# sashakolpakov/graphem-rapids

Measured on AMD Instinct MI355X. Metric: layout iterations/s, higher is better.
Workload: dtype f32

## Files before the change

graphem-rapids_amd/_native.py:

```python
import ctypes
import os

import numpy as np

_HERE = os.path.dirname(os.path.abspath(__file__))
LIB_PATH = os.path.join(_HERE, "libgraphem_hip.so")

GH_OK, GH_ERR_INVALID, GH_ERR_RUNTIME, GH_ERR_K_TOO_LARGE, GH_ERR_HIP, GH_ERR_NOMEM = range(6)

SYMBOLS = [
    "gh_create", "gh_destroy", "gh_last_error", "gh_set_positions", "gh_get_positions", "gh_positions_device",
    "gh_row_stride", "gh_step", "gh_run", "gh_sync", "gh_spring_forces", "gh_knn_midpoints",
    "gh_intersection_forces", "gh_integrate_normalise", "gh_step_begin", "gh_knn_partial_device", "gh_knn_partial_cols", "gh_knn_merged_device", "gh_rows_packed_device", "gh_step_unpack_rows", "gh_set_packed_rows", "gh_step_merge",
    "gh_stats_partial_device", "gh_step_finish", "gh_timing_enable", "gh_timing_reset", "gh_timing_count",
    "gh_timing_get", "gh_device_count", "gh_version", "gh_knn_last_counts", "gh_set_stream",
    "gh_positions_rows_allocated", "gh_knn_points", "gh_stats_rows", "gh_spmv_symnorm",
    "gh_spectral_last_error", "gh_gather_layout", "gh_gather_buffer_device", "gh_gather_slot_bytes",
    "gh_step_finish_gathered", "gh_vertex_order", "gh_positions_unpadded_device", "gh_radial_topk",
    "gh_comm_unique_id", "gh_comm_init_rccl", "gh_loopback_group_create", "gh_loopback_group_destroy",
    "gh_comm_init_loopback", "gh_comm_destroy", "gh_run_partitioned", "gh_comm_last_error", "gh_debug_stamps",
    "gh_knn_cdist_stats", "gh_rank_layout", "gh_step_finish_own", "gh_comm_available", "gh_selftest_arith",
    "gh_create_f64", "gh_set_positions_f64", "gh_get_positions_f64", "gh_positions_device_f64", "gh_spring_forces_f64",
    "gh_intersection_forces_f64", "gh_trlan_sweep", "gh_knn_ivf_config", "gh_knn_ivf_list_sizes",
    "gh_torch_randperm_prefix", "gh_torch_randperm_isa", "gh_run_torch_sampled", "gh_set_cdist_replay", "gh_sampler_stats",
    "gh_overlap_layout", "gh_rows_all_device", "gh_rows_all_row_floats", "gh_stats_all_device", "gh_stats_all_block_doubles", "gh_step_rows_early",
    "gh_step_pack_rows", "gh_step_finish_overlap",
    "gh_ic_create", "gh_ic_destroy", "gh_ic_last_error", "gh_ic_arc_count", "gh_ic_set_memory_budget", "gh_ic_spread",
]


class GhParams(ctypes.Structure):
    _fields_ = [("L_min", ctypes.c_float), ("k_attr", ctypes.c_float), ("k_inter", ctypes.c_float),
                ("n_neighbors", ctypes.c_int32), ("sample_size", ctypes.c_int32), ("seed", ctypes.c_uint64),
                ("reorder", ctypes.c_int32), ("knn_method", ctypes.c_int32), ("knn_distance", ctypes.c_int32),
                ("ivf_lists", ctypes.c_int32), ("ivf_probes", ctypes.c_int32)]


REORDER = {"auto": 0, "off": 1, "bfs": 2}
KNN_METHOD = {"auto": 0, "scan": 1, "grid": 2, "ivf": 3}
KNN_DISTANCE = {"exact": 0, "cdist": 1}


class GhPartition(ctypes.Structure):
    _fields_ = [("row_lo", ctypes.c_int64), ("row_hi", ctypes.c_int64),
                ("edge_lo", ctypes.c_int64), ("edge_hi", ctypes.c_int64), ("edge_rule", ctypes.c_int32)]


EDGES_RANGE, EDGES_HASHED = 0, 1


_lib = None


def load():
    global _lib
    if _lib is not None:
        return _lib
    global LIB_PATH
    if os.environ.get("GRAPHEM_HIP_LIB"):
        LIB_PATH = os.environ["GRAPHEM_HIP_LIB"]
    if not os.path.exists(LIB_PATH):
        raise RuntimeError(
            f"{LIB_PATH} is missing: build it with `python graphem-rapids_amd/build.py` "
            "(hipcc --offload-arch=gfx950). The HIP backend has no CPU fallback.")
# ... 109 lines not shown
    L.gh_trlan_sweep.restype = ctypes.c_int
    L.gh_spectral_last_error.argtypes = []
    L.gh_spectral_last_error.restype = ctypes.c_char_p
    L.gh_stats_rows.argtypes = [vp]
    L.gh_stats_rows.restype = i32
    L.gh_knn_points.argtypes = [ctypes.c_int, vp, i64, vp, i64, i32, i32, vp]
    L.gh_knn_points.restype = ctypes.c_int
    L.gh_knn_last_counts.argtypes = [vp, vp, vp, vp]
    L.gh_knn_last_counts.restype = ctypes.c_int
    L.gh_knn_cdist_stats.argtypes = [vp, vp, vp]
    L.gh_knn_cdist_stats.restype = ctypes.c_int
    L.gh_sampler_stats.argtypes = [vp, vp]
    L.gh_sampler_stats.restype = ctypes.c_int
    L.gh_set_cdist_replay.argtypes = [vp, i32]
    L.gh_set_cdist_replay.restype = ctypes.c_int
    L.gh_knn_ivf_config.argtypes = [vp, vp, vp]
    L.gh_knn_ivf_config.restype = ctypes.c_int
    L.gh_knn_ivf_list_sizes.argtypes = [vp, vp, ctypes.c_int32]
    L.gh_knn_ivf_list_sizes.restype = ctypes.c_int
    L.gh_comm_unique_id.argtypes = [vp]
    L.gh_comm_unique_id.restype = ctypes.c_int
    L.gh_comm_init_rccl.argtypes = [vp, i32, i32, vp]
    L.gh_comm_init_rccl.restype = ctypes.c_int
    L.gh_loopback_group_create.argtypes = [i32]
    L.gh_loopback_group_create.restype = vp
    L.gh_loopback_group_destroy.argtypes = [vp]
    L.gh_loopback_group_destroy.restype = None
    L.gh_comm_init_loopback.argtypes = [vp, vp, i32]
    L.gh_comm_init_loopback.restype = ctypes.c_int
    L.gh_comm_destroy.argtypes = [vp]
# ... 283 lines not shown
        return self.lib.gh_stats_partial_device(self.handle)

    def knn_last_counts(self):
        a, b, c = (np.zeros(self.S, dtype=np.int32) for _ in range(3))
        self._chk(self.lib.gh_knn_last_counts(self.handle, ptr(a), ptr(b), ptr(c)))
        return a, b, c

    def knn_cdist_stats(self):
        a, b = ctypes.c_int32(0), ctypes.c_int32(0)
        self._chk(self.lib.gh_knn_cdist_stats(self.handle, ctypes.byref(a), ctypes.byref(b)))
        return a.value, b.value

    def set_cdist_replay(self, all_ties):
        self._chk(self.lib.gh_set_cdist_replay(self.handle, 1 if all_ties else 0))

    def knn_ivf_config(self):
        a, b = ctypes.c_int32(0), ctypes.c_int32(0)
        self._chk(self.lib.gh_knn_ivf_config(self.handle, ctypes.byref(a), ctypes.byref(b)))
        return a.value, b.value

    def knn_ivf_list_sizes(self):
        out = np.zeros(self.knn_ivf_config()[0], dtype=np.int32)
        self._chk(self.lib.gh_knn_ivf_list_sizes(self.handle, ptr(out), len(out)))
        return out

    def timing_enable(self, on=True):
        self._chk(self.lib.gh_timing_enable(self.handle, 1 if on else 0))

    def timing_reset(self):
        self._chk(self.lib.gh_timing_reset(self.handle))
# ... 105 lines not shown
```

graphem-rapids_amd/csrc/api.hip:

```cpp
#include "common.h"
#include "engine.h"

#include "torch_randperm.h"

#include <algorithm>
#include <chrono>
#include <condition_variable>
#include <mutex>
#include <new>
#include <thread>
#include <stdlib.h>
#include <string.h>

static thread_local std::string g_create_error;
void gh_set_create_error(const std::string &msg) { g_create_error = msg; }

gh_scope::gh_scope(gh_engine *h_, const char *name, hipStream_t on) : h(h_), stream(on ? on : h_->stream) {
    if (!h->timing) return;
    for (size_t i = 0; i < h->timers.size(); ++i)
        if (h->timers[i].name == name) slot = (int)i;
    if (slot < 0) {
        h->timers.emplace_back();
        h->timers.back().name = name;
        slot = (int)h->timers.size() - 1;
// ... 49 lines not shown
    }
    return GH_OK;
}

static gh_status reject_f64(gh_engine *h, const char *what) {
    if (!h->f64) return GH_OK;
    h->err = std::string(what) + " is not available on a float64 engine";
    return GH_ERR_INVALID;
}

static void free_all(gh_engine *h) {
    gh_f64_free(h);
    gh_ivf_free(h);
    void *ptrs[] = {h->d_edges, h->d_rowptr, h->d_adj, h->d_pos, (h->d_gbuf || h->d_rows_all) ? (void *)h->d_new_own : (void *)h->d_new, h->d_gbuf, h->d_rows_all, h->d_rows_pk, h->d_stats_all, h->d_tmpF, h->d_tmpF2, h->d_io, h->d_acc,
                    h->d_tflag, h->d_touched, h->d_tcount, h->d_sampled, h->d_q, h->d_qscan, h->d_qA, h->d_qexact, h->d_order, h->d_long_rows, h->d_long_ownptr, h->d_long_ownadj, h->d_long_eptr, h->d_long_erow, h->d_long_terms, h->d_own_long, h->d_cand, h->d_cnt,
                    h->d_ovf, h->d_sel_redo, h->d_tq_count, h->d_tq_base, h->d_tq_touched, h->d_dbg_cnt, h->d_partial, h->d_merged, h->d_first_edge, h->d_own_eids, h->d_mid, h->d_Fs, h->d_gmin, h->d_sub_uv, h->d_stamps, h->d_tau_flag, h->d_wait_failed, h->d_grid_u32, h->d_grid_smid, h->d_grid_temp, h->d_stats_comb, h->d_rows_packed, h->d_rare, h->d_cd_rows, h->d_cd_vbuf, h->d_cd_cmin, h->d_cd_stat, h->d_vblock, h->d_blockstats, (h->d_gbuf || h->d_rows_all) ? (void *)h->d_stats_own : (void *)h->d_stats, h->d_iscratch, h->d_stream_ids};
    for (void *p : ptrs)
        if (p) (void)hipFree(p);
    if (h->h_ring) (void)hipHostFree(h->h_ring);
    for (hipEvent_t e : h->ring_ev)
        if (e) (void)hipEventDestroy(e);
    if (h->own_stream) (void)hipStreamDestroy(h->own_stream);
}

gh_status gh_check_create_args(int device_id, int64_t n, int32_t D, int64_t E, const int32_t *edges, const gh_params *params,
                               int f64_max_D, double f64_k_attr) {
    auto fail = [&](gh_status st, const std::string &msg) { g_create_error = msg; return st; };
    const bool f64 = f64_max_D > 0;
    if (n <= 0) return fail(GH_ERR_INVALID, "Adjacency matrix cannot be empty");
    if (D <= 0) return fail(GH_ERR_INVALID, "Number of components must be positive, got " + std::to_string(D));
    if (f64 && D > f64_max_D) return fail(GH_ERR_INVALID, "the float64 engine takes up to " + std::to_string(f64_max_D) + " components");
// ... 97 lines not shown
    if (!up(h->d_edges, g.edges, sizeof(int32_t) * 2 * (size_t)E) || !up32(h->d_rowptr, g.rowptr) ||
        !up(h->d_adj, g.adj.data(), sizeof(int32_t) * (size_t)h->adj_len) || !up32(h->d_first_edge, g.first_edge) ||
        !up32(h->d_vblock, g.vblock) || (hashed && !up32(h->d_own_eids, g.own_eids)) ||
        (h->nlong && (!up32(h->d_long_rows, g.long_rows) || !up32(h->d_long_ownptr, g.long_ownptr) ||
                      !up32(h->d_long_eptr, g.long_eptr) || !up32(h->d_long_erow, g.long_erow) ||
                      !up32(h->d_long_ownadj, g.long_ownadj) || !up(h->d_own_long, g.own_long.data(), g.own_long.size()))) ||
        hipStreamSynchronize(h->stream) != hipSuccess) {
        h->err = "upload of the graph failed";
        return GH_ERR_HIP;
    }
    GH_TRY(gh_grid_alloc(h));
    GH_TRY(gh_ivf_alloc(h));
    GH_TRY(gh_cdist_alloc(h));
    GH_A(d_tau_flag, 1, true);
    GH_A(d_wait_failed, 1, true);
    if (sw.stamps) GH_A(d_stamps, ((size_t)std::max(h->n_vblocks, 1) + GH_STAMP_EXTRA) * 8, true);
#undef GH_A
    if (h->thr_M1 > 0 && hipMemcpy(h->d_sub_uv, g.sub_uv.data(), sizeof(int32_t) * g.sub_uv.size(), hipMemcpyHostToDevice) != hipSuccess) {
        h->err = "upload of the threshold subset failed";
        return GH_ERR_HIP;
    }
    if (!h->order_host.empty()) {
        GH_TRY(dev_alloc(h, &h->d_order, (size_t)n, false));
        if (hipMemcpy(h->d_order, h->order_host.data(), sizeof(int32_t) * (size_t)n, hipMemcpyHostToDevice) != hipSuccess) {
            h->err = "upload of the vertex order failed";
            return GH_ERR_HIP;
        }
    }
    return GH_OK;
}
// ... 29 lines not shown
    h->rows = h->part.row_hi - h->part.row_lo;

    auto bail = [&](gh_status st) { g_create_error = h->err; free_all(h); delete h; return st; };
    if (hipSetDevice(device_id) != hipSuccess) return bail(GH_ERR_HIP);
    if (hipStreamCreateWithFlags(&h->own_stream, hipStreamNonBlocking) != hipSuccess) { h->err = "hipStreamCreate failed"; return bail(GH_ERR_HIP); }
    h->stream = h->own_stream;
    h->pos_rows = n + GH_POS_PAD_ROWS;
    const create_switches sw = read_switches();
    h->opt_no_presetup = sw.no_presetup;

    gh_graph_plan g;
    gh_plan_graph(h, edges, part != nullptr, sw.reorder ? atoi(sw.reorder) : params->reorder, &g);
    if (auto_method) gh_auto_knn_method(h);
    gh_choose_threshold_subset(h);
    gh_plan_threshold_subset(h, &g);
    h->tau_embedded = sw.tau_separate >= 0 ? sw.tau_separate == 0 : h->n_vblocks <= 2048;

    const gh_status st = allocate_and_upload(h, g, sw);
    if (st != GH_OK) return bail(st);
    *out = h;
    return GH_OK;
}

extern "C" void gh_destroy(gh_handle h) {
    if (!h) return;
    (void)hipSetDevice(h->device);
    (void)hipStreamSynchronize(h->stream);
    resolve_timers(h);
    gh_comm_free(h);
    free_all(h);
    delete h;
// ... 8 lines not shown
    gh_set_lookahead(h, nullptr);
    GH_HIP(hipMemcpyAsync(h->d_io, pos, sizeof(float) * (size_t)h->n * h->D, hipMemcpyHostToDevice, h->stream));
    GH_TRY(gh_launch_pad(h, h->d_io, h->d_pos));
    GH_HIP(hipStreamSynchronize(h->stream));
    return GH_OK;
}

static gh_status download_padded(gh_engine *h, const float *d_src, float *host) {
    GH_TRY(gh_launch_unpad(h, d_src, h->d_io));
    GH_HIP(hipMemcpyAsync(host, h->d_io, sizeof(float) * (size_t)h->n * h->D, hipMemcpyDeviceToHost, h->stream));
    GH_HIP(hipStreamSynchronize(h->stream));
    return GH_OK;
}

static gh_status check_device_waits(gh_engine *h) {
    if (!h->tau_embedded || !h->d_wait_failed) return GH_OK;
    int32_t failed = 0;
    GH_HIP(hipMemcpyAsync(&failed, h->d_wait_failed, sizeof(failed), hipMemcpyDeviceToHost, h->stream));
    GH_HIP(hipStreamSynchronize(h->stream));
    if (failed) {
        GH_HIP(hipMemsetAsync(h->d_wait_failed, 0, sizeof(int32_t), h->stream));
        GH_HIP(hipStreamSynchronize(h->stream));
        h->tau_embedded = false;
        h->err = "a workgroup of the fused spring+scan launch timed out waiting for the thresholds of its own launch; "
                 "results since the last successful gh_sync / gh_get_positions are invalid -- set the positions again. "
                 "The engine now computes the thresholds in a launch of their own (as GRAPHEM_HIP_TAU_SEPARATE=1 does); "
                 "please report this";
        return GH_ERR_RUNTIME;
    }
    return GH_OK;
}

extern "C" gh_status gh_get_positions(gh_handle h, float *pos) {
    GH_TRY(check_handle(h));
    if (h->f64) return pos ? gh_f64_get_positions_f32(h, pos) : GH_ERR_INVALID;
    if (!pos) { h->err = "positions is NULL"; return GH_ERR_INVALID; }
    GH_TRY(check_device_waits(h));
    return download_padded(h, h->d_pos, pos);
// ... 159 lines not shown
    if (iters == 0) return GH_OK;
    GH_TRY(check_whole(h, "gh_run"));
    GH_TRY(check_k(h));
    int32_t *d_ids = nullptr;
    GH_TRY(gh_upload_sample_stream(h, iters, sample_stream, &d_ids));
    const gh_ids own = gh_own_ids(h);
    auto src = [&](int32_t t) { return d_ids ? gh_ids{GH_IDS_GIVEN, d_ids + (size_t)t * h->S} : own; };
    return run_iterations(h, iters, d_ids == nullptr, src, nothing_before);
}

extern "C" gh_status gh_set_cdist_replay(gh_handle h, int32_t all_ties) {
    GH_TRY(check_handle(h));
    GH_TRY(reject_f64(h, "gh_set_cdist_replay"));
    if (!h->cdist) { h->err = "gh_set_cdist_replay: not a GH_DIST_CDIST engine"; return GH_ERR_INVALID; }
    h->cd_all_ties = all_ties != 0;
    return GH_OK;
}

extern "C" gh_status gh_torch_randperm_prefix(uint8_t *rng_state, int64_t state_bytes, int64_t n, int64_t S, int32_t iters,
                                              int32_t *ids) {
    if (!rng_state || state_bytes != GH_TORCH_RNG_STATE_BYTES || n < 0 || n >= ((int64_t)1 << 31) || S < 0 || S > n || iters < 0 ||
        (!ids && iters > 0 && S > 0))
        return GH_ERR_INVALID;
    gh_mt19937 mt;
    if (!gh_mt_load(&mt, rng_state)) return GH_ERR_INVALID;
    std::vector<int64_t> scratch((size_t)gh_rp_scratch_words(S));
    for (int32_t t = 0; t < iters; ++t) gh_torch_randperm_prefix_one(&mt, n, S, ids + (size_t)t * (size_t)S, scratch.data());
    gh_mt_store(&mt, rng_state);
    return GH_OK;
}
// ... 481 lines not shown
```

graphem-rapids_amd/csrc/engine.h:

```cpp
#pragma once
#include <hip/hip_runtime.h>
#include <stdint.h>
#include <string>
#include <vector>

#include "../../include/graphem_hip.h"

#define GH_CAND_CAP 16384
#define GH_SEL_BUF 4096
#define GH_SEL_CHUNK 2048
#define GH_CNT_STRIDE 32
#define GH_POS_PAD_ROWS 1024
inline int gh_fix_blocks(int LD) { return LD <= 16 ? 2 * LD : 0; }
#define GH_SCAN_MIN_EDGES 16384

struct gh_timer_slot {
    std::string name;
    double total_ms = 0.0;
    int64_t launches = 0;
    std::vector<std::pair<hipEvent_t, hipEvent_t>> pending;
};

enum { GH_IDS_GIVEN = 0, GH_IDS_SAMPLER = 1, GH_IDS_ARANGE = 2 };
struct gh_ids {
// ... 129 lines not shown

    int grid_G = 0, grid_bits = 0;
    int64_t grid_cells = 0;
    size_t grid_temp_bytes = 0;
    uint32_t *d_grid_u32 = nullptr;
    void *d_grid_smid = nullptr;
    void *d_grid_temp = nullptr;

    gh_ivf *ivf = nullptr;

    double *d_blockstats = nullptr;
    int nblocks_update = 0;
    double *d_stats = nullptr;

    bool tau_embedded = false;
    unsigned *d_tau_flag = nullptr;
    int32_t *d_wait_failed = nullptr;

#define GH_STAMP_EXTRA 8192
    unsigned long long *d_stamps = nullptr;
    bool timing = false;
    std::vector<gh_timer_slot> timers;
};

inline gh_ids gh_own_ids(const gh_engine *h) { return gh_ids{h->S >= h->E ? GH_IDS_ARANGE : GH_IDS_SAMPLER, h->d_sampled}; }
inline void gh_set_lookahead(gh_engine *h, const gh_ids *next) {
    h->lookahead.valid = next != nullptr;
    if (next) { h->lookahead.src = *next; h->lookahead.iter = h->iter + 1; }
}

struct gh_scope {
// ... 50 lines not shown
                               int D, int K, uint64_t *d_keys, std::string *err);
gh_status gh_cdist_alloc(gh_engine *h);
gh_status gh_knn_merge_cdist(gh_engine *h, const uint64_t *gathered, int world);
gh_status gh_knn_finish_cdist(gh_engine *h, bool all_rows, bool fuse_intersect);
bool gh_grid_path(const gh_engine *h);
gh_status gh_grid_alloc(gh_engine *h);
gh_status gh_grid_search(gh_engine *h);
bool gh_ivf_path(const gh_engine *h);
gh_status gh_ivf_alloc(gh_engine *h);
void gh_ivf_free(gh_engine *h);
gh_status gh_ivf_search(gh_engine *h);
gh_status gh_radial_topk_device(gh_engine *h, int K, uint64_t *d_part, int nparts, int32_t *d_ids);
int gh_fused_mfma_kb(const gh_engine *h);
bool gh_fused_uses_mfma(const gh_engine *h);
int gh_fused_tile(const gh_engine *h);
gh_status gh_launch_spring_scan(gh_engine *h);
gh_status gh_knn_merge(gh_engine *h, const uint64_t *gathered, int world);
gh_status gh_launch_intersect(gh_engine *h);
gh_status gh_launch_inter_cleanup(gh_engine *h);
gh_status gh_launch_spring_mid(gh_engine *h);
gh_status gh_launch_mid_only(gh_engine *h);
gh_status gh_launch_integrate(gh_engine *h);
gh_status gh_launch_spring_only(gh_engine *h, float *d_F);
gh_status gh_launch_inter_to_dense(gh_engine *h, float *d_F);
gh_status gh_launch_integrate_given(gh_engine *h, const float *d_Fs, const float *d_Fi);
gh_status gh_launch_normalise(gh_engine *h, bool with_cleanup, const gh_ids *next = nullptr);
gh_status gh_launch_normalise_gathered(gh_engine *h, const gh_ids *next);
gh_status gh_launch_normalise_own(gh_engine *h, const double *stats_all, int world);
gh_status gh_launch_unpack_rows(gh_engine *h);
struct gh_long_args;
// ... 37 lines not shown
```

graphem-rapids_amd/csrc/fused.hip:

```cpp
#include "common.h"
#include "engine.h"
#include "scan_core.h"
#include "tau_core.h"

#include <stdio.h>
#include <stdlib.h>

static bool fused_mfma(int LD, int D, int64_t S) {
    (void)S;
    return D <= 16 && (LD == 4 || LD == 8 || LD == 16);
}
static int fused_mfma_kb(int LD, int D, int64_t S) { return fused_mfma(LD, D, S) && D <= 3 ? 0 : -1; }
static void fused_cfg(int LD, int D, int64_t S, int64_t own_edges, int *nt, int *r) {
    (void)LD; (void)D; (void)S; (void)own_edges;
    *nt = 256;
    *r = 2;
}
bool gh_fused_uses_mfma(const gh_engine *h) { return h->fused_scan && fused_mfma(h->LD, h->D, h->S); }
int gh_fused_mfma_kb(const gh_engine *h) { return h->fused_scan ? fused_mfma_kb(h->LD, h->D, h->S) : -1; }
int gh_fused_tile(const gh_engine *h) {
    int nt, r;
    fused_cfg(h->LD, h->D, h->S, h->own_count, &nt, &r);
    return nt * r;
}

namespace {

template <int D, int LD, int NT, bool LONG>
__device__ __forceinline__ void gh_phase_a(const float *__restrict__ pos, const int32_t *__restrict__ rowptr,
                                           const int32_t *__restrict__ adj, const int32_t *__restrict__ first_edge,
                                           int v0, int v1, int fe0, int nedges, int64_t row_lo, float L_min, float neg_k,
                                           float *__restrict__ Fs, float *__restrict__ out_new, float *mids,
                                           double (&sx)[LD], double (&sxx)[LD], const gh_long_args &la,
                                           const float *__restrict__ Fpre = nullptr ) {
// ... 210 lines not shown
        const int nb_ = nbad;
        for (int p = threadIdx.x; p < nb_ * nq; p += NT) {
            const int s = p % nq;
            const gh_h8 hi = qa[2 * s + 1];
            if ((float)hi[4] == GH_MF_NEVER) continue;
            park(s_lo, s, badlist[p / nq]);
        }
    }
    __syncthreads();
    GH_STAMP(4);
    gh_flush_hits<HITBUF, NT>(hkey, hq, &hcount, cand, cnt);
    GH_STAMP(5);
#undef GH_STAMP
}

template <int D, int LD, bool LONG>
__global__ __launch_bounds__(256) void spring_scan_mfmaw_kernel(
    const float *__restrict__ pos, const int32_t *__restrict__ rowptr, const int32_t *__restrict__ adj,
    const int32_t *__restrict__ first_edge, const int32_t *__restrict__ own_eids,
    const int32_t *__restrict__ vblock, int64_t row_lo, float L_min, float neg_k, float *__restrict__ Fs,
    float *__restrict__ out_new, double *__restrict__ blockstats, const float *__restrict__ qt,
    const float *__restrict__ qscan, int S,
    uint64_t *__restrict__ cand, int32_t *__restrict__ cnt, gh_long_args la, gh_tau_args ta,
    unsigned long long *__restrict__ stamps) {
    constexpr int NT = 256, R = 2, TILE = NT * R, NB = 2 * R;
    constexpr int HITBUF = LD == 16 ? 256 : 512;
    constexpr int KB = D <= 10 ? 1 : 2;
    constexpr int QS = LD + 4, QT = LD;
    if ((int)blockIdx.x < ta.nblocks) {
        if (blockIdx.y == 0) gh_tau_produce<NT, -1>(ta, stamps ? stamps + ((int64_t)gridDim.x - 2 * ta.nblocks + GH_STAMP_EXTRA + blockIdx.x) * 8 : nullptr);
// ... 195 lines not shown
    ta.cdist = h->cdist ? 1 : 0;
    ta.flag = h->d_tau_flag;
    ta.target = (unsigned)h->S;
    ta.nblocks = gh_tau_blocks((int)h->S, nt);
    ta.wait_failed = h->d_wait_failed;
    return ta;
}

template <int D, int R, bool DEFER>
void launch_mfma_d(gh_engine *h) {
    const gh_tau_args ta = fused_tau_args(h, 256);
    spring_scan_mfma_kernel<D, R, DEFER><<<dim3(fused_grid(h, ta)), dim3(256), 0, h->stream>>>(
        h->d_pos, h->d_rowptr, h->d_adj, h->d_first_edge, h->d_own_eids, h->d_vblock, h->part.row_lo, h->prm.L_min,
        -h->prm.k_attr, h->d_Fs, h->d_new, h->d_blockstats, h->d_q, reinterpret_cast<const gh_h8 *>(h->d_qA),
        h->d_qexact, (int)h->S, h->d_cand, h->d_cnt, gh_make_long_args(h, true), ta, h->d_stamps);
}
template <int D, int R>
void launch_mfma(gh_engine *h) {
    if (R == 2 && h->n_vblocks <= 2048) launch_mfma_d<D, R, (R == 2)>(h);
    else launch_mfma_d<D, R, false>(h);
}

template <int D, int LD, bool LONG>
void launch_mfmaw_l(gh_engine *h) {
    unsigned ny = 1;
    if (h->n_vblocks < 384) {
        static int resident = 0;
        if (resident == 0) {
            int occ = 0, cus = 0;
            if (hipOccupancyMaxActiveBlocksPerMultiprocessor(&occ, spring_scan_mfmaw_kernel<D, LD, LONG>, 256, 0) != hipSuccess) occ = 1;
// ... 27 lines not shown
        switch (h->D) {
            case 4: launch_mfmaw<4, 4>(h); break;
            case 5: launch_mfmaw<5, 8>(h); break;
            case 6: launch_mfmaw<6, 8>(h); break;
            case 7: launch_mfmaw<7, 8>(h); break;
            case 8: launch_mfmaw<8, 8>(h); break;
            case 9: launch_mfmaw<9, 16>(h); break;
            case 10: launch_mfmaw<10, 16>(h); break;
            case 11: launch_mfmaw<11, 16>(h); break;
            case 12: launch_mfmaw<12, 16>(h); break;
            case 13: launch_mfmaw<13, 16>(h); break;
            case 14: launch_mfmaw<14, 16>(h); break;
            case 15: launch_mfmaw<15, 16>(h); break;
            default: launch_mfmaw<16, 16>(h); break;
        }
    } else if (fused_mfma(h->LD, h->D, h->S)) {
        if (h->D == 2) launch_mfma<2, 2>(h); else launch_mfma<3, 2>(h);
    } else {
        h->err = "fused spring+scan launched for an unsupported dimension";
        return GH_ERR_RUNTIME;
    }
    GH_LAUNCH_CHECK();
    h->new0_ready = true;
    return GH_OK;
}
```

include/graphem_hip.h:

```cpp
#ifndef GRAPHEM_HIP_H
#define GRAPHEM_HIP_H

#include <stdint.h>

#ifdef __cplusplus
extern "C" {
#endif

typedef struct gh_engine *gh_handle;

typedef enum {
    GH_OK = 0,
    GH_ERR_INVALID = 1,
    GH_ERR_RUNTIME = 2,
    GH_ERR_K_TOO_LARGE = 3,
    GH_ERR_HIP = 4,
    GH_ERR_NOMEM = 5
} gh_status;

typedef struct {
    float L_min;
    float k_attr;
    float k_inter;
    int32_t n_neighbors;
// ... 107 lines not shown
gh_status gh_run_partitioned(gh_handle h, int32_t iters, const int32_t *sample_stream);
const char *gh_comm_last_error(void);


gh_status gh_timing_enable(gh_handle h, int32_t on);
gh_status gh_timing_reset(gh_handle h);
int32_t gh_timing_count(gh_handle h);
gh_status gh_timing_get(gh_handle h, int32_t i, const char **name, double *total_ms, int64_t *launches);


gh_status gh_debug_stamps(gh_handle h, unsigned long long *out, int64_t count);

gh_status gh_knn_last_counts(gh_handle h, int32_t *subset_counts, int32_t *final_counts, int32_t *overflow);
gh_status gh_knn_cdist_stats(gh_handle h, int32_t *full_pass_rows, int32_t *unresolved_tie_rows);
gh_status gh_set_cdist_replay(gh_handle h, int32_t all_ties);
gh_status gh_knn_ivf_config(gh_handle h, int32_t *lists, int32_t *probes);
gh_status gh_knn_ivf_list_sizes(gh_handle h, int32_t *sizes, int32_t count);

gh_status gh_knn_points(int device_id, const float *q, int64_t nq, const float *ref, int64_t nref,
                        int32_t n_components, int32_t k, int64_t *out);

gh_status gh_radial_topk(gh_handle h, int32_t k, int32_t *ids);

gh_status gh_spmv_symnorm(void *hip_stream, int64_t n, const int64_t *indptr, const int32_t *indices,
                          const double *inv_sqrt_deg, const double *x, double *y);
gh_status gh_trlan_sweep(void *hip_stream, int64_t n, const int64_t *indptr, const int32_t *indices,
                         const double *inv_sqrt_deg, double *V, int32_t nl, int32_t m, int32_t k, double *Td,
                         double *work, double *beta, double *hmax);
const char *gh_spectral_last_error(void);

// ... 21 lines not shown
```

Baseline: 6062.

## Add query-cell spatial filter to fused spring+scan kernel

Adds a fused spring+scan kernel variant. Block 0 builds a small 8-per-axis grid of quantile-bounded cells over the sampled queries and publishes it to global memory. Every other workgroup waits on an epoch flag, loads the table into shared memory, and tests each midpoint only against the queries listed in its cell plus a 'wide' list, instead of running the split-f16 MFMA pre-filter against all queries. It is picked automatically when tau is not embedded and D<=3, S<=256. It adds a cross-workgroup spin-wait with a timeout fallback, and it risks imbalance when many queries land in the wide list.

```diff
diff --git a/graphem-rapids_amd/_native.py b/graphem-rapids_amd/_native.py
--- a/graphem-rapids_amd/_native.py
+++ b/graphem-rapids_amd/_native.py
@@ -22,7 +22,7 @@
     "gh_knn_cdist_stats", "gh_rank_layout", "gh_step_finish_own", "gh_comm_available", "gh_selftest_arith",
     "gh_create_f64", "gh_set_positions_f64", "gh_get_positions_f64", "gh_positions_device_f64", "gh_spring_forces_f64",
     "gh_intersection_forces_f64", "gh_trlan_sweep", "gh_knn_ivf_config", "gh_knn_ivf_list_sizes",
-    "gh_torch_randperm_prefix", "gh_torch_randperm_isa", "gh_run_torch_sampled", "gh_set_cdist_replay", "gh_sampler_stats",
+    "gh_torch_randperm_prefix", "gh_torch_randperm_isa", "gh_run_torch_sampled", "gh_set_cdist_replay", "gh_set_scan_filter", "gh_get_scan_filter", "gh_qcell_probe", "gh_sampler_stats",
     "gh_overlap_layout", "gh_rows_all_device", "gh_rows_all_row_floats", "gh_stats_all_device", "gh_stats_all_block_doubles", "gh_step_rows_early",
     "gh_step_pack_rows", "gh_step_finish_overlap",
     "gh_ic_create", "gh_ic_destroy", "gh_ic_last_error", "gh_ic_arc_count", "gh_ic_set_memory_budget", "gh_ic_spread",
@@ -48,6 +48,8 @@
 
 EDGES_RANGE, EDGES_HASHED = 0, 1
 
+
+SCAN_FILTERS = {"auto": 0, "mfma": 1, "cells": 2}
 
 _lib = None
 
@@ -187,6 +189,12 @@
     L.gh_sampler_stats.restype = ctypes.c_int
     L.gh_set_cdist_replay.argtypes = [vp, i32]
     L.gh_set_cdist_replay.restype = ctypes.c_int
+    L.gh_set_scan_filter.argtypes = [vp, i32]
+    L.gh_set_scan_filter.restype = ctypes.c_int
+    L.gh_get_scan_filter.argtypes = [vp, ctypes.POINTER(i32)]
+    L.gh_get_scan_filter.restype = ctypes.c_int
+    L.gh_qcell_probe.argtypes = [vp, i32, vp, vp, vp, i64, vp, vp]
+    L.gh_qcell_probe.restype = ctypes.c_int
     L.gh_knn_ivf_config.argtypes = [vp, vp, vp]
     L.gh_knn_ivf_config.restype = ctypes.c_int
     L.gh_knn_ivf_list_sizes.argtypes = [vp, vp, ctypes.c_int32]
@@ -500,6 +508,14 @@
     def set_cdist_replay(self, all_ties):
         self._chk(self.lib.gh_set_cdist_replay(self.handle, 1 if all_ties else 0))
 
+    def set_scan_filter(self, mode):
+        self._chk(self.lib.gh_set_scan_filter(self.handle, SCAN_FILTERS[mode]))
+
+    def scan_filter(self):
+        v = ctypes.c_int32(0)
+        self._chk(self.lib.gh_get_scan_filter(self.handle, ctypes.byref(v)))
+        return {b: a for a, b in SCAN_FILTERS.items()}[v.value]
+
     def knn_ivf_config(self):
         a, b = ctypes.c_int32(0), ctypes.c_int32(0)
         self._chk(self.lib.gh_knn_ivf_config(self.handle, ctypes.byref(a), ctypes.byref(b)))
diff --git a/graphem-rapids_amd/csrc/api.hip b/graphem-rapids_amd/csrc/api.hip
--- a/graphem-rapids_amd/csrc/api.hip
+++ b/graphem-rapids_amd/csrc/api.hip
@@ -1,5 +1,6 @@
 #include "common.h"
 #include "engine.h"
+#include "qcell_core.h"
 
 #include "torch_randperm.h"
 
@@ -87,7 +88,7 @@
     gh_ivf_free(h);
     void *ptrs[] = {h->d_edges, h->d_rowptr, h->d_adj, h->d_pos, (h->d_gbuf || h->d_rows_all) ? (void *)h->d_new_own : (void *)h->d_new, h->d_gbuf, h->d_rows_all, h->d_rows_pk, h->d_stats_all, h->d_tmpF, h->d_tmpF2, h->d_io, h->d_acc,
                     h->d_tflag, h->d_touched, h->d_tcount, h->d_sampled, h->d_q, h->d_qscan, h->d_qA, h->d_qexact, h->d_order, h->d_long_rows, h->d_long_ownptr, h->d_long_ownadj, h->d_long_eptr, h->d_long_erow, h->d_long_terms, h->d_own_long, h->d_cand, h->d_cnt,
-                    h->d_ovf, h->d_sel_redo, h->d_tq_count, h->d_tq_base, h->d_tq_touched, h->d_dbg_cnt, h->d_partial, h->d_merged, h->d_first_edge, h->d_own_eids, h->d_mid, h->d_Fs, h->d_gmin, h->d_sub_uv, h->d_stamps, h->d_tau_flag, h->d_wait_failed, h->d_grid_u32, h->d_grid_smid, h->d_grid_temp, h->d_stats_comb, h->d_rows_packed, h->d_rare, h->d_cd_rows, h->d_cd_vbuf, h->d_cd_cmin, h->d_cd_stat, h->d_vblock, h->d_blockstats, (h->d_gbuf || h->d_rows_all) ? (void *)h->d_stats_own : (void *)h->d_stats, h->d_iscratch, h->d_stream_ids};
+                    h->d_ovf, h->d_sel_redo, h->d_tq_count, h->d_tq_base, h->d_tq_touched, h->d_dbg_cnt, h->d_partial, h->d_merged, h->d_first_edge, h->d_own_eids, h->d_mid, h->d_Fs, h->d_gmin, h->d_sub_uv, h->d_stamps, h->d_tau_flag, h->d_wait_failed, h->d_qcell, h->d_qc_flag, h->d_grid_u32, h->d_grid_smid, h->d_grid_temp, h->d_stats_comb, h->d_rows_packed, h->d_rare, h->d_cd_rows, h->d_cd_vbuf, h->d_cd_cmin, h->d_cd_stat, h->d_vblock, h->d_blockstats, (h->d_gbuf || h->d_rows_all) ? (void *)h->d_stats_own : (void *)h->d_stats, h->d_iscratch, h->d_stream_ids};
     for (void *p : ptrs)
         if (p) (void)hipFree(p);
     if (h->h_ring) (void)hipHostFree(h->h_ring);
@@ -215,6 +216,8 @@
     GH_TRY(gh_cdist_alloc(h));
     GH_A(d_tau_flag, 1, true);
     GH_A(d_wait_failed, 1, true);
+    GH_A(d_qcell, GH_QC_WORDS, true);
+    GH_A(d_qc_flag, 1, true);
     if (sw.stamps) GH_A(d_stamps, ((size_t)std::max(h->n_vblocks, 1) + GH_STAMP_EXTRA) * 8, true);
 #undef GH_A
     if (h->thr_M1 > 0 && hipMemcpy(h->d_sub_uv, g.sub_uv.data(), sizeof(int32_t) * g.sub_uv.size(), hipMemcpyHostToDevice) != hipSuccess) {
@@ -274,7 +277,8 @@
     if (auto_method) gh_auto_knn_method(h);
     gh_choose_threshold_subset(h);
     gh_plan_threshold_subset(h, &g);
-    h->tau_embedded = sw.tau_separate >= 0 ? sw.tau_separate == 0 : h->n_vblocks <= 2048;
+    h->tau_embedded_plan = sw.tau_separate >= 0 ? sw.tau_separate == 0 : h->n_vblocks <= 2048;
+    gh_choose_scan_filter(h);
 
     const gh_status st = allocate_and_upload(h, g, sw);
     if (st != GH_OK) return bail(st);
@@ -313,14 +317,24 @@
 }
 
 static gh_status check_device_waits(gh_engine *h) {
-    if (!h->tau_embedded || !h->d_wait_failed) return GH_OK;
+    if (!(h->tau_embedded || h->qcells) || !h->d_wait_failed) return GH_OK;
     int32_t failed = 0;
     GH_HIP(hipMemcpyAsync(&failed, h->d_wait_failed, sizeof(failed), hipMemcpyDeviceToHost, h->stream));
     GH_HIP(hipStreamSynchronize(h->stream));
     if (failed) {
         GH_HIP(hipMemsetAsync(h->d_wait_failed, 0, sizeof(int32_t), h->stream));
         GH_HIP(hipStreamSynchronize(h->stream));
-        h->tau_embedded = false;
+        if (h->qcells) {
+            h->scan_filter = GH_FILTER_MFMA;
+            gh_choose_scan_filter(h);
+            h->lookahead.valid = false;
+            h->err = "a workgroup of the fused spring+scan launch timed out waiting for the query-cell table of its own "
+                     "launch; results since the last successful gh_sync / gh_get_positions are invalid -- set the positions "
+                     "again.  The engine now uses the split-f16 pre-filter (GH_FILTER_MFMA); please report this";
+            return GH_ERR_RUNTIME;
+        }
+        h->tau_embedded_plan = false;
+        gh_choose_scan_filter(h);
         h->err = "a workgroup of the fused spring+scan launch timed out waiting for the thresholds of its own launch; "
                  "results since the last successful gh_sync / gh_get_positions are invalid -- set the positions again. "
                  "The engine now computes the thresholds in a launch of their own (as GRAPHEM_HIP_TAU_SEPARATE=1 does); "
@@ -510,6 +524,52 @@
     GH_TRY(reject_f64(h, "gh_set_cdist_replay"));
     if (!h->cdist) { h->err = "gh_set_cdist_replay: not a GH_DIST_CDIST engine"; return GH_ERR_INVALID; }
     h->cd_all_ties = all_ties != 0;
+    return GH_OK;
+}
+
+extern "C" gh_status gh_set_scan_filter(gh_handle h, int32_t mode) {
+    GH_TRY(check_handle(h));
+    GH_TRY(reject_f64(h, "gh_set_scan_filter"));
+    if (mode != GH_FILTER_AUTO && mode != GH_FILTER_MFMA && mode != GH_FILTER_CELLS) {
+        h->err = "gh_set_scan_filter: mode must be GH_FILTER_AUTO, GH_FILTER_MFMA or GH_FILTER_CELLS";
+        return GH_ERR_INVALID;
+    }
+    if (mode == GH_FILTER_CELLS && !gh_fused_cells_ok(h)) {
+        h->err = "gh_set_scan_filter: the query-cell filter needs a fused engine with n_components <= 3 and 1 <= sample_size <= " +
+                 std::to_string(GH_QC_SMAX);
+        return GH_ERR_INVALID;
+    }
+    h->scan_filter = mode;
+    const bool was_embedded = h->tau_embedded;
+    gh_choose_scan_filter(h);
+    if (h->tau_embedded != was_embedded) h->lookahead.valid = false;
+    return GH_OK;
+}
+
+extern "C" gh_status gh_get_scan_filter(gh_handle h, int32_t *mode) {
+    GH_TRY(check_handle(h));
+    if (!mode) { h->err = "mode is NULL"; return GH_ERR_INVALID; }
+    *mode = h->f64 || !gh_fused_uses_mfma(h) || h->D > 3 ? GH_FILTER_AUTO : h->qcells ? GH_FILTER_CELLS : GH_FILTER_MFMA;
+    return GH_OK;
+}
+
+extern "C" gh_status gh_qcell_probe(const float *bounds, int32_t D, const float *q, const float *tau, const float *m, int64_t n,
+                                    float *d2, int32_t *cells) {
+    if (!bounds || !q || !tau || !m || !d2 || !cells || D < 1 || D > 3 || n < 0) return GH_ERR_INVALID;
+    for (int64_t i = 0; i < n; ++i) {
+        float acc = 0.0f;
+        for (int d = 0; d < D; ++d) {
+            const float df = q[i * D + d] - m[i * D + d];
+            acc = fmaf(df, df, acc);
+            const float *b = bounds + d * (GH_QC_G - 1);
+            int lo, hi;
+            gh_qc_axis_box(b, q[i * D + d], tau[i], lo, hi);
+            cells[(i * D + d) * 3] = gh_qc_axis_cell(b, m[i * D + d]);
+            cells[(i * D + d) * 3 + 1] = lo;
+            cells[(i * D + d) * 3 + 2] = hi;
+        }
+        d2[i] = acc;
+    }
     return GH_OK;
 }
 
diff --git a/graphem-rapids_amd/csrc/engine.h b/graphem-rapids_amd/csrc/engine.h
--- a/graphem-rapids_amd/csrc/engine.h
+++ b/graphem-rapids_amd/csrc/engine.h
@@ -167,7 +167,13 @@
     double *d_stats = nullptr;
 
     bool tau_embedded = false;
+    bool tau_embedded_plan = false;
     unsigned *d_tau_flag = nullptr;
+    int scan_filter = 0;
+    bool qcells = false;
+    uint32_t *d_qcell = nullptr;
+    unsigned *d_qc_flag = nullptr;
+    unsigned qc_epoch = 0;
     int32_t *d_wait_failed = nullptr;
 
 #define GH_STAMP_EXTRA 8192
@@ -248,6 +254,8 @@
 int gh_fused_mfma_kb(const gh_engine *h);
 bool gh_fused_uses_mfma(const gh_engine *h);
 int gh_fused_tile(const gh_engine *h);
+bool gh_fused_cells_ok(const gh_engine *h);
+void gh_choose_scan_filter(gh_engine *h);
 gh_status gh_launch_spring_scan(gh_engine *h);
 gh_status gh_knn_merge(gh_engine *h, const uint64_t *gathered, int world);
 gh_status gh_launch_intersect(gh_engine *h);
diff --git a/graphem-rapids_amd/csrc/fused.hip b/graphem-rapids_amd/csrc/fused.hip
--- a/graphem-rapids_amd/csrc/fused.hip
+++ b/graphem-rapids_amd/csrc/fused.hip
@@ -1,5 +1,6 @@
 #include "common.h"
 #include "engine.h"
+#include "qcell_core.h"
 #include "scan_core.h"
 #include "tau_core.h"
 
@@ -17,7 +18,15 @@
     *r = 2;
 }
 bool gh_fused_uses_mfma(const gh_engine *h) { return h->fused_scan && fused_mfma(h->LD, h->D, h->S); }
-int gh_fused_mfma_kb(const gh_engine *h) { return h->fused_scan ? fused_mfma_kb(h->LD, h->D, h->S) : -1; }
+int gh_fused_mfma_kb(const gh_engine *h) { return h->fused_scan && !h->qcells ? fused_mfma_kb(h->LD, h->D, h->S) : -1; }
+bool gh_fused_cells_ok(const gh_engine *h) {
+    return h->fused_scan && fused_mfma(h->LD, h->D, h->S) && h->D <= 3 && h->S >= 1 && h->S <= GH_QC_SMAX;
+}
+void gh_choose_scan_filter(gh_engine *h) {
+    const bool want = h->scan_filter == GH_FILTER_CELLS || (h->scan_filter == GH_FILTER_AUTO && !h->tau_embedded_plan);
+    h->qcells = want && gh_fused_cells_ok(h);
+    h->tau_embedded = h->tau_embedded_plan && !h->qcells;
+}
 int gh_fused_tile(const gh_engine *h) {
     int nt, r;
     fused_cfg(h->LD, h->D, h->S, h->own_count, &nt, &r);
@@ -258,6 +267,145 @@
 #undef GH_STAMP
 }
 
+template <int D>
+__global__ __launch_bounds__(256) void spring_scan_cells_kernel(
+    const float *__restrict__ pos, const int32_t *__restrict__ rowptr, const int32_t *__restrict__ adj,
+    const int32_t *__restrict__ first_edge, const int32_t *__restrict__ own_eids,
+    const int32_t *__restrict__ vblock, int64_t row_lo, float L_min, float neg_k, float *__restrict__ Fs,
+    float *__restrict__ out_new, double *__restrict__ blockstats, const float *__restrict__ qt, int S,
+    uint32_t *__restrict__ qcell, unsigned *__restrict__ qc_flag, unsigned epoch, int32_t *__restrict__ wait_failed,
+    uint64_t *__restrict__ cand, int32_t *__restrict__ cnt, gh_long_args la, int cdist, unsigned long long *__restrict__ stamps) {
+    constexpr int LD = 4, NT = 256, R = 2, TILE = NT * R, HITBUF = 512;
+    static_assert(D <= 3, "query records of one 16-byte load");
+    __shared__ float4 tile[TILE];
+    __shared__ float4 qrec[GH_QC_SMAX];
+    __shared__ uint32_t tab[GH_QC_WORDS];
+    __shared__ uint64_t hkey[HITBUF];
+    __shared__ int hq[HITBUF];
+    __shared__ uint32_t ids[TILE];
+    __shared__ int hcount;
+    if (blockIdx.x == 0) {
+        gh_qc_build<D, NT>(reinterpret_cast<const float4 *>(qt), S, tab, qrec, reinterpret_cast<uint32_t *>(hkey));
+        for (int i = threadIdx.x; i < GH_QC_WORDS; i += NT)
+            __hip_atomic_store(qcell + i, tab[i], __ATOMIC_RELAXED, __HIP_MEMORY_SCOPE_AGENT);
+        asm volatile("s_waitcnt vmcnt(0)" ::: "memory");
+        __syncthreads();
+        if (threadIdx.x == 0) __hip_atomic_store(qc_flag, epoch, __ATOMIC_RELAXED, __HIP_MEMORY_SCOPE_AGENT);
+        return;
+    }
+    const int nbx = (int)gridDim.x - 1;
+    const int bx = (int)blockIdx.x - 1;
+#define GH_STAMP(k) do { if (stamps && threadIdx.x == 0) stamps[(int64_t)bx * 8 + (k)] = wall_clock64(); } while (0)
+    GH_STAMP(0);
+    if (stamps && threadIdx.x == 0) { stamps[(int64_t)bx * 8 + 6] = vblock[bx + 1] - vblock[bx]; stamps[(int64_t)bx * 8 + 7] = first_edge[vblock[bx + 1]] - first_edge[vblock[bx]]; }
+    float *mids = reinterpret_cast<float *>(tile);
+    const int v0 = vblock[bx], v1 = vblock[bx + 1];
+    const int fe0 = first_edge[v0];
+    const int nedges = first_edge[v1] - fe0;
+    if (threadIdx.x == 0) hcount = 0;
+    for (int j = threadIdx.x; j < nedges; j += NT) ids[j] = own_eids ? (uint32_t)own_eids[fe0 + j] : (uint32_t)(fe0 + j);
+
+    const int t_idle = min(NT, (v1 - v0 + 63) / 64 * 64);
+    auto stage = [&](int t0) {
+        for (int i = (int)threadIdx.x - t0; i < S; i += NT - t0) qrec[i] = reinterpret_cast<const float4 *>(qt)[i];
+        unsigned spins = 0;
+        while ((int)(__hip_atomic_load(qc_flag, __ATOMIC_RELAXED, __HIP_MEMORY_SCOPE_AGENT) - epoch) < 0) {
+            __builtin_amdgcn_s_sleep(32);
+            if (++spins > (1u << 20)) { *wait_failed = 1; break; }
+        }
+        __builtin_amdgcn_fence(__ATOMIC_ACQUIRE, "wavefront");
+        for (int i = (int)threadIdx.x - t0; i < GH_QC_WORDS / 4; i += NT - t0)
+            reinterpret_cast<float4 *>(tab)[i] = gh_ld_f4(reinterpret_cast<const float4 *>(qcell) + i, true);
+    };
+    if (t_idle < NT && (int)threadIdx.x >= t_idle) stage(t_idle);
+
+    __shared__ double red[(NT / 64) * 2 * LD];
+    {
+        double sx[LD], sxx[LD];
+        gh_phase_a<D, LD, NT, true>(pos, rowptr, adj, first_edge, v0, v1, fe0, nedges, row_lo, L_min, neg_k, Fs, out_new, mids, sx, sxx, la);
+        GH_STAMP(1);
+        gh_block_stats<LD, NT>(sx, sxx, red, blockstats, bx, nbx, v1 - v0);
+    }
+    GH_STAMP(2);
+    if (t_idle == NT) {
+        stage(0);
+        __syncthreads();
+    }
+    GH_STAMP(3);
+
+    const float *bnd = reinterpret_cast<const float *>(tab + GH_QC_OFF_B);
+    const uint16_t *ptr = reinterpret_cast<const uint16_t *>(tab + GH_QC_OFF_PTR);
+    const uint8_t *ent = reinterpret_cast<const uint8_t *>(tab + GH_QC_OFF_ENT);
+    const uint8_t *wide = reinterpret_cast<const uint8_t *>(tab + GH_QC_OFF_WIDE);
+    const int nwide = (int)tab[GH_QC_OFF_NWIDE];
+    auto park = [&](int s, const float4 qr, int j, const float (&m)[3]) {
+        const float q[3] = {qr.x, qr.y, qr.z};
+        float d2 = 0.0f;
+#pragma unroll
+        for (int d = 0; d < D; ++d) {
+            const float df = q[d] - m[d];
+            d2 = fmaf(df, df, d2);
+        }
+        if (d2 <= qr.w) {
+            if (cdist) d2 = gh_aten_cdist<D>(q, m);
+            const uint32_t id = ids[j];
+            const int p = atomicAdd(&hcount, 1);
+            if (p < HITBUF) { hkey[p] = gh_key(d2, id); hq[p] = s; }
+            else gh_append_candidate(cand, cnt, s, gh_key(d2, id));
+        }
+    };
+    constexpr int U = 4;
+    float m[R][3];
+    int e[R], e1[R];
+#pragma unroll
+    for (int r = 0; r < R; ++r) {
+        const int j = (int)threadIdx.x + r * NT;
+        const float4 mv = tile[j < nedges ? j : 0];
+        m[r][0] = mv.x; m[r][1] = mv.y; m[r][2] = mv.z;
+        int c = gh_qc_axis_cell(bnd, m[r][0]) + GH_QC_G * gh_qc_axis_cell(bnd + 8, m[r][1]);
+        if constexpr (D == 3) c += GH_QC_G * GH_QC_G * gh_qc_axis_cell(bnd + 16, m[r][2]);
+        e[r] = j < nedges ? ptr[c] : 0;
+        e1[r] = j < nedges ? ptr[c + 1] : 0;
+    }
+#pragma unroll
+    for (int r = 0; r < R; ++r) {
+        const int j = (int)threadIdx.x + r * NT;
+        for (int b = e[r]; b < e1[r]; b += U) {
+            int s[U];
+            float4 qr[U];
+#pragma unroll
+            for (int u = 0; u < U; ++u) s[u] = ent[min(b + u, e1[r] - 1)];
+#pragma unroll
+            for (int u = 0; u < U; ++u) qr[u] = qrec[s[u]];
+#pragma unroll
+            for (int u = 0; u < U; ++u)
+                if (b + u < e1[r]) park(s[u], qr[u], j, m[r]);
+        }
+    }
+    for (int b = 0; b < nwide; b += U) {
+        int s[U];
+        float4 qr[U];
+#pragma unroll
+        for (int u = 0; u < U; ++u) s[u] = wide[min(b + u, nwide - 1)];
+#pragma unroll
+        for (int u = 0; u < U; ++u) qr[u] = qrec[s[u]];
+#pragma unroll
+        for (int r = 0; r < R; ++r) {
+            const int j = (int)threadIdx.x + r * NT;
+            if (j < nedges) {
+#pragma unroll
+                for (int u = 0; u < U; ++u)
+                    if (b + u < nwide) park(s[u], qr[u], j, m[r]);
+            }
+        }
+    }
+    __syncthreads();
+    GH_STAMP(4);
+    gh_flush_hits<HITBUF, NT>(hkey, hq, &hcount, cand, cnt);
+    GH_STAMP(5);
+#undef GH_STAMP
+}
+
 template <int D, int LD, bool LONG>
 __global__ __launch_bounds__(256) void spring_scan_mfmaw_kernel(
     const float *__restrict__ pos, const int32_t *__restrict__ rowptr, const int32_t *__restrict__ adj,
@@ -483,6 +631,14 @@
         h->d_pos, h->d_rowptr, h->d_adj, h->d_first_edge, h->d_own_eids, h->d_vblock, h->part.row_lo, h->prm.L_min,
         -h->prm.k_attr, h->d_Fs, h->d_new, h->d_blockstats, h->d_q, reinterpret_cast<const gh_h8 *>(h->d_qA),
         h->d_qexact, (int)h->S, h->d_cand, h->d_cnt, gh_make_long_args(h, true), ta, h->d_stamps);
+}
+template <int D>
+void launch_cells(gh_engine *h) {
+    if (++h->qc_epoch == 0) h->qc_epoch = 1;
+    spring_scan_cells_kernel<D><<<dim3((unsigned)h->n_vblocks + 1), dim3(256), 0, h->stream>>>(
+        h->d_pos, h->d_rowptr, h->d_adj, h->d_first_edge, h->d_own_eids, h->d_vblock, h->part.row_lo, h->prm.L_min,
+        -h->prm.k_attr, h->d_Fs, h->d_new, h->d_blockstats, h->d_q, (int)h->S, h->d_qcell, h->d_qc_flag, h->qc_epoch,
+        h->d_wait_failed, h->d_cand, h->d_cnt, gh_make_long_args(h, true), h->cdist ? 1 : 0, h->d_stamps);
 }
 template <int D, int R>
 void launch_mfma(gh_engine *h) {
@@ -540,6 +696,8 @@
             case 15: launch_mfmaw<15, 16>(h); break;
             default: launch_mfmaw<16, 16>(h); break;
         }
+    } else if (h->qcells) {
+        if (h->D == 2) launch_cells<2>(h); else launch_cells<3>(h);
     } else if (fused_mfma(h->LD, h->D, h->S)) {
         if (h->D == 2) launch_mfma<2, 2>(h); else launch_mfma<3, 2>(h);
     } else {
diff --git a/graphem-rapids_amd/csrc/qcell_core.h b/graphem-rapids_amd/csrc/qcell_core.h
--- /dev/null
+++ b/graphem-rapids_amd/csrc/qcell_core.h
@@ -0,0 +1,144 @@
+#pragma once
+#include "common.h"
+
+#define GH_QC_G 8
+#define GH_QC_CAP 27
+#define GH_QC_ENT 2048
+#define GH_QC_SMAX 256
+#define GH_QC_CELLS (GH_QC_G * GH_QC_G * GH_QC_G)
+#define GH_QC_SAMPLE 64
+#define GH_QC_OFF_NWIDE 0
+#define GH_QC_OFF_B 4
+#define GH_QC_OFF_PTR 28
+#define GH_QC_OFF_ENT 288
+#define GH_QC_OFF_WIDE (GH_QC_OFF_ENT + GH_QC_ENT / 4)
+#define GH_QC_WORDS (GH_QC_OFF_WIDE + GH_QC_SMAX / 4)
+static_assert(GH_QC_OFF_B + 3 * 8 <= GH_QC_OFF_PTR, "blob layout");
+static_assert(GH_QC_OFF_PTR + (GH_QC_CELLS + 2) / 2 <= GH_QC_OFF_ENT, "blob layout");
+static_assert(GH_QC_WORDS % 4 == 0, "the blob moves in 16-byte pieces");
+
+__host__ __device__ inline int gh_qc_axis_cell(const float *b, float x) {
+    int c = 0;
+#pragma unroll
+    for (int i = 0; i < GH_QC_G - 1; ++i) c += b[i] <= x ? 1 : 0;
+    return c;
+}
+
+__host__ __device__ inline void gh_qc_axis_box(const float *b, float q, float tau, int &lo, int &hi) {
+    lo = 0;
+    hi = 0;
+#pragma unroll
+    for (int i = 0; i < GH_QC_G - 1; ++i) {
+        const float df = q - b[i];
+        const bool far = fmaf(df, df, 0.0f) > tau;
+        if (b[i] <= q) { lo += far ? 1 : 0; hi += 1; }
+        else hi += far ? 0 : 1;
+    }
+}
+
+template <int NT>
+__device__ __forceinline__ uint32_t gh_qc_block_scan(uint32_t v, uint32_t *wsum , uint32_t &total) {
+    const int lane = threadIdx.x & 63, w = threadIdx.x >> 6;
+    uint32_t incl = v;
+#pragma unroll
+    for (int o = 1; o < 64; o <<= 1) {
+        const uint32_t x = __shfl_up(incl, o, 64);
+        if (lane >= o) incl += x;
+    }
+    __syncthreads();
+    if (lane == 63) wsum[w] = incl;
+    __syncthreads();
+    uint32_t base = 0;
+    total = 0;
+#pragma unroll
+    for (int ww = 0; ww < NT / 64; ++ww) {
+        base += ww < w ? wsum[ww] : 0;
+        total += wsum[ww];
+    }
+    return base + incl - v;
+}
+
+template <int D, int NT>
+__device__ __forceinline__ void gh_qc_build(const float4 *__restrict__ qt, int S, uint32_t *tab, float4 *rec, uint32_t *cnt) {
+    static_assert(NT >= GH_QC_SMAX, "one query per thread");
+    constexpr int NC = D == 3 ? GH_QC_CELLS : GH_QC_G * GH_QC_G;
+    const int t = threadIdx.x;
+    float4 r = make_float4(0.f, 0.f, 0.f, -1.f);
+    if (t < S) { r = qt[t]; rec[t] = r; }
+    for (int c = t; c < NC; c += NT) cnt[c] = 0;
+    if (t == 0) tab[GH_QC_OFF_NWIDE] = 0;
+    __syncthreads();
+    float *bnd = reinterpret_cast<float *>(tab + GH_QC_OFF_B);
+    const int w = t >> 6, lane = t & 63;
+    if (w < D) {
+        const int n = min(S, GH_QC_SAMPLE);
+        const float4 sr = lane < n ? rec[(int)(((int64_t)lane * S) / n)] : make_float4(0.f, 0.f, 0.f, 0.f);
+        const float x = w == 0 ? sr.x : w == 1 ? sr.y : sr.z;
+        const uint32_t u = __float_as_uint(x);
+        const uint32_t key = lane < n ? ((u & 0x80000000u) ? ~u : (u | 0x80000000u)) : 0xFFFFFFFFu;
+        int rank = 0;
+        for (int p = 0; p < n; ++p) {
+            const uint32_t kp = (uint32_t)__builtin_amdgcn_readlane((int)key, p);
+            rank += (kp < key || (kp == key && p < lane)) ? 1 : 0;
+        }
+        if (lane < n) {
+#pragma unroll
+            for (int i = 1; i < GH_QC_G; ++i)
+                if (rank == (i * n) / GH_QC_G) bnd[w * 8 + i - 1] = x;
+        }
+    }
+    __syncthreads();
+    __shared__ uint32_t wsum[NT / 64];
+    int lo[3] = {0, 0, 0}, hi[3] = {0, 0, 0};
+    bool listed = false;
+    int ncell = 0;
+    uint8_t *wide = reinterpret_cast<uint8_t *>(tab + GH_QC_OFF_WIDE);
+    if (t < S) {
+        const float q[3] = {r.x, r.y, r.z};
+        bool finite = isfinite(r.w);
+        ncell = 1;
+#pragma unroll
+        for (int d = 0; d < D; ++d) {
+            finite = finite && isfinite(q[d]);
+            gh_qc_axis_box(bnd + d * 8, q[d], r.w, lo[d], hi[d]);
+            ncell *= hi[d] - lo[d] + 1;
+        }
+        listed = finite && ncell <= GH_QC_CAP;
+    }
+    {
+        uint32_t total;
+        const uint32_t before = gh_qc_block_scan<NT>(listed ? (uint32_t)ncell : 0u, wsum, total);
+        listed = listed && before + (uint32_t)ncell <= GH_QC_ENT;
+    }
+    if (t < S && !listed) wide[atomicAdd(&tab[GH_QC_OFF_NWIDE], 1u)] = (uint8_t)t;
+    const int wx = hi[0] - lo[0] + 1, wy = hi[1] - lo[1] + 1;
+    auto cell_of = [&](int k) {
+        const int x = k % wx, y = (k / wx) % wy, z = k / (wx * wy);
+        return (lo[0] + x) + GH_QC_G * ((lo[1] + y) + GH_QC_G * (lo[2] + z));
+    };
+    if (listed)
+        for (int k = 0; k < ncell; ++k) atomicAdd(&cnt[cell_of(k)], 1u);
+    __syncthreads();
+    uint16_t *ptr = reinterpret_cast<uint16_t *>(tab + GH_QC_OFF_PTR);
+    {
+        static_assert(GH_QC_CELLS <= 2 * NT, "two cells per thread");
+        const uint32_t a = 2 * t < NC ? cnt[2 * t] : 0, b = 2 * t + 1 < NC ? cnt[2 * t + 1] : 0;
+        uint32_t total;
+        const uint32_t ex = gh_qc_block_scan<NT>(a + b, wsum, total);
+        if (2 * t < NC) { ptr[2 * t] = (uint16_t)ex; cnt[2 * t] = ex; }
+        if (2 * t + 1 < NC) { ptr[2 * t + 1] = (uint16_t)(ex + a); cnt[2 * t + 1] = ex + a; }
+        if (t == 0) ptr[NC] = (uint16_t)total;
+    }
+    __syncthreads();
+    uint8_t *ent = reinterpret_cast<uint8_t *>(tab + GH_QC_OFF_ENT);
+    if (listed)
+        for (int k0 = 0; k0 < ncell; k0 += 4) {
+            uint32_t at[4];
+#pragma unroll
+            for (int u = 0; u < 4; ++u) at[u] = k0 + u < ncell ? atomicAdd(&cnt[cell_of(k0 + u)], 1u) : 0u;
+#pragma unroll
+            for (int u = 0; u < 4; ++u)
+                if (k0 + u < ncell) ent[at[u]] = (uint8_t)t;
+        }
+    __syncthreads();
+}
diff --git a/include/graphem_hip.h b/include/graphem_hip.h
--- a/include/graphem_hip.h
+++ b/include/graphem_hip.h
@@ -145,6 +145,13 @@
 gh_status gh_knn_last_counts(gh_handle h, int32_t *subset_counts, int32_t *final_counts, int32_t *overflow);
 gh_status gh_knn_cdist_stats(gh_handle h, int32_t *full_pass_rows, int32_t *unresolved_tie_rows);
 gh_status gh_set_cdist_replay(gh_handle h, int32_t all_ties);
+#define GH_FILTER_AUTO 0
+#define GH_FILTER_MFMA 1
+#define GH_FILTER_CELLS 2
+gh_status gh_set_scan_filter(gh_handle h, int32_t mode);
+gh_status gh_get_scan_filter(gh_handle h, int32_t *mode);
+gh_status gh_qcell_probe(const float *bounds, int32_t D, const float *q, const float *tau, const float *m, int64_t n,
+                         float *d2, int32_t *cells);
 gh_status gh_knn_ivf_config(gh_handle h, int32_t *lists, int32_t *probes);
 gh_status gh_knn_ivf_list_sizes(gh_handle h, int32_t *sizes, int32_t count);
 
```

Measured after the change: 6512, median of 6. 1.07x the previous value.
